# pfnet-research/superpixel-align

Measured on AMD Instinct MI355X. Metric: images/sec superpixel-align labelling (1024x2048), higher is better.
Workload: dtype f32 as 2 x f16 planes, f32 accumulate

## Files before the change

### include/spalign.h

```cpp
#ifndef SPALIGN_H
#define SPALIGN_H

#include <stddef.h>
#include <stdint.h>

#ifdef __cplusplus
extern "C" {
#endif

#define SPA_OK 0
#define SPA_ERR_ARG (-1)
#define SPA_ERR_HIP (-2)
#define SPA_ERR_NOGPU (-3)
#define SPA_ERR_LAYOUT (-4)
#define SPA_ERR_CAPACITY (-5)

#define SPA_ST_SLIC_EMPTY_SEGMENT 0x01u
#define SPA_ST_SLIC_UNCOVERED 0x02u
#define SPA_ST_CONN_OVERSIZE 0x04u
#define SPA_ST_POOL_SLOT_OVERFLOW 0x08u
#define SPA_ST_KMEANS_BARRIER 0x10u
#define SPA_ST_LABEL_RANGE 0x20u
#define SPA_ST_RNG_UNDERRUN 0x40u
#define SPA_ST_NP_SHUFFLE 0x80u

#define SPA_CELL_SLOTS 16

typedef struct spa_ctx spa_ctx;

int spa_version(void);
const char *spa_last_error(void);
int spa_ctx_create(int device, spa_ctx **out);
void spa_ctx_destroy(spa_ctx *ctx);
int spa_status(spa_ctx *ctx, uint32_t *status_host, void *stream);
int spa_status_peek_async(spa_ctx *ctx, uint32_t *status_pinned, void *stream);
int spa_status_take_async(spa_ctx *ctx, uint32_t *status_pinned, void *stream);

int spa_prof_enable(spa_ctx *ctx, int on);
int spa_prof_slots(void);
const char *spa_prof_name(int slot);
int spa_prof_read(spa_ctx *ctx, int slot, double *total_ms_host, int *launches_host);
int spa_debug_peek(spa_ctx *ctx, int which, size_t offset, size_t bytes, void *host);
int spa_ws_generation(spa_ctx *ctx);
int spa_debug_set(spa_ctx *ctx, int32_t key, int32_t value);
int spa_wino4_tile_decode(int32_t B, int32_t H, int32_t W, int32_t dilation, int32_t interleaved, int64_t t, int32_t *out);
int spa_debug_lds_probe(spa_ctx *ctx, float *out, int32_t n_wg, int32_t steps, int32_t mode, void *stream);

int spa_drn_normalise(spa_ctx *ctx, const float *x, int32_t B, int32_t H, int32_t W, void *out,
                      int32_t out_dtype, const double *mean3_host, const double *std3_host, void *stream);
int spa_bias_act(spa_ctx *ctx, void *y, int32_t dtype, int64_t rows, int32_t C, const void *bias,
                 const void *residual, int32_t relu, void *stream);
int spa_bias_act_amax(spa_ctx *ctx, float *y, int64_t rows, int32_t C, const float *bias,
                      const float *residual, int32_t relu, void *amax, void *stream);

int spa_drn_stem_d(spa_ctx *ctx, const float *x, int32_t B, int32_t H, int32_t W,
                   const float *w0, const float *b0, const float *w1, const float *b1,
                   const double *mean3_host, const double *std3_host, void *y, int32_t out_dtype,
                   float *xn_scratch, void *stream);

int spa_conv3x3_bf16(spa_ctx *ctx, const void *x, int32_t B, int32_t H, int32_t W, int32_t Cin,
                     const void *wt, int32_t Cout, const float *bias, const void *residual,
                     int32_t relu, int32_t dilation, void *y, void *stream);

int spa_conv_bf16_light(spa_ctx *ctx, const void *x, int32_t B, int32_t Hi, int32_t Wi, int32_t Cin, const void *wt,
                        int32_t taps, int32_t stride, int32_t Cout, const float *bias, const void *residual,
                        int32_t relu, int32_t dilation, void *y, void *stream);

// ... 306 lines not shown
```

### superpixel-align_amd/_lib.py

```python
import ctypes
import os
import subprocess

_HERE = os.path.dirname(os.path.abspath(__file__))
LIB_PATH = os.environ.get('SPA_LIB_PATH') or os.path.join(_HERE, 'libspalign.so')
_LIB = None

SPA_OK = 0
STATUS_BITS = {
    0x01: 'SLIC: a seed lost all of its pixels (NaN centre, dead for the rest of the sweeps, as in scikit-image)',
    0x02: 'SLIC: a pixel fell outside every 2S search window',
    0x04: 'connectivity: a component reached max_size (cut in BFS order by the exact replay path)',
    0x08: 'mean pooling: more than 16 superpixels touch one feature pixel',
    0x10: 'k-means: grid barrier timed out',
    0x20: 'a superpixel label outside [0, n_labels) was met',
    0x40: 'anchor selection: the device random stream ran dry',
    0x80: 'k-means initial assignment on the device: more than 65 536 points at or below the median weight',
}

INFO_BITS = 0x01 | 0x04

c_i32 = ctypes.c_int32
c_i64 = ctypes.c_int64
c_f32 = ctypes.c_float
# ... 35 lines not shown
    'spa_conv3x3_f32': (ctypes.c_int, [c_p, c_p, c_i32, c_i32, c_i32, c_i32, c_p, c_i32, c_p, c_p, c_i32, c_i32, c_p, c_p]),
    'spa_conv1x1_f32': (ctypes.c_int, [c_p, c_p, c_i32, c_i32, c_i32, c_i32, c_p, c_i32, c_p, c_p, c_i32, c_p, c_p]),
    'spa_wino_tiles': (ctypes.c_int64, [c_i32, c_i32, c_i32, c_i32]),
    'spa_conv3x3_wino_f32': (ctypes.c_int, [c_p, c_p, c_i32, c_i32, c_i32, c_i32, c_p, c_i32, c_p, c_p, c_i32, c_i32, c_p, c_p, c_p, c_p]),
    'spa_wino4_tiles': (ctypes.c_int64, [c_i32, c_i32, c_i32, c_i32]),
    'spa_conv3x3_wino4_f32': (ctypes.c_int, [c_p, c_p, c_i32, c_i32, c_i32, c_i32, c_p, c_i32, c_p, c_p, c_i32, c_i32, c_p, c_p, c_p, c_p]),
    'spa_conv3x3_f16s': (ctypes.c_int, [c_p, c_p, c_i32, c_i32, c_i32, c_i32, c_p, c_f32, c_i32, c_p, c_p, c_i32, c_i32, c_p, c_p, c_p, c_p]),
    'spa_conv1x1_f16s': (ctypes.c_int, [c_p, c_p, c_i32, c_i32, c_i32, c_i32, c_p, c_f32, c_i32, c_p, c_p, c_i32, c_p, c_p, c_p, c_p]),
    'spa_conv3x3_s2_f16s': (ctypes.c_int, [c_p, c_p, c_i32, c_i32, c_i32, c_i32, c_p, c_f32, c_i32, c_i32, c_p, c_i32, c_p, c_p, c_p, c_p, c_p]),
    'spa_bias_act_amax': (ctypes.c_int, [c_p, c_p, c_i64, c_i32, c_p, c_p, c_i32, c_p, c_p]),
    'spa_drn_stem_d_amax': (ctypes.c_int, [c_p, c_p, c_i32, c_i32, c_i32, c_p, c_p, c_p, c_p, c_p, c_p, c_p, c_p, c_p, c_p]),
    'spa_drn_stem_c_amax': (ctypes.c_int, [c_p, c_p, c_i32, c_i32, c_i32, c_p, c_p, c_p, c_p, c_p, c_p, c_p, c_p, c_p, c_p, c_p]),
    'spa_drn_stem_c_bf16': (ctypes.c_int, [c_p, c_p, c_i32, c_i32, c_i32, c_p, c_p, c_p, c_p, c_p, c_p, c_p, c_p, c_p, c_p]),
    'spa_conv_small_f16s': (ctypes.c_int, [c_p, c_p, c_i32, c_i32, c_i32, c_i32, c_p, c_f32, c_i32, c_i32, c_i32, c_p, c_p, c_i32, c_p, c_p, c_p, c_p, c_p]),
    'spa_drn_layer2_f16s': (ctypes.c_int, [c_p, c_p, c_i32, c_i32, c_i32, c_p, c_f32, c_p, c_p, c_p, c_p, c_p]),
    'spa_drn_layer2_f32': (ctypes.c_int, [c_p, c_p, c_i32, c_i32, c_i32, c_p, c_p, c_p, c_p]),
    'spa_conv3x3_s2_f32': (ctypes.c_int, [c_p, c_p, c_i32, c_i32, c_i32, c_i32, c_p, c_i32, c_i32, c_p, c_i32, c_p, c_p, c_p]),
    'spa_amax_f32': (ctypes.c_int, [c_p, c_p, c_i64, c_p, c_p]),
    'spa_conv3x3_wino4_f16s': (ctypes.c_int, [c_p, c_p, c_i32, c_i32, c_i32, c_i32, c_p, c_p, c_i32, c_p, c_p, c_i32, c_i32, c_p, c_p, c_p, c_p, c_p, c_p]),
    'spa_resize_bicubic_u8': (ctypes.c_int, [c_p, c_p, c_i32, c_i32, c_i32, c_i32, c_i32, c_i32, c_p, c_p]),
    'spa_resize_cvcubic_u8': (ctypes.c_int, [c_p, c_p, c_i32, c_i32, c_i32, c_i32, c_i32, c_i32, c_p, c_p]),
    'spa_debug_peek': (ctypes.c_int, [c_p, ctypes.c_int, ctypes.c_size_t, ctypes.c_size_t, c_p]),
    'spa_debug_set': (ctypes.c_int, [c_p, ctypes.c_int32, ctypes.c_int32]),
    'spa_wino4_tile_decode': (ctypes.c_int, [c_i32, c_i32, c_i32, c_i32, c_i32, c_i64, ctypes.POINTER(ctypes.c_int32)]),
    'spa_ws_generation': (ctypes.c_int, [c_p]),
    'spa_debug_lds_probe': (ctypes.c_int, [c_p, c_p, c_i32, c_i32, c_i32, c_p]),
    'spa_slic_make_plan':(ctypes.c_int, [c_i32, c_i32, c_i32, ctypes.POINTER(SlicPlan)]),
    'spa_rgb2lab': (ctypes.c_int, [c_p, c_p, c_i32, c_i32, c_i32, c_f32, c_p, c_p]),
    'spa_slic_core': (ctypes.c_int, [c_p, c_p, c_i32, c_i32, c_i32, c_i32, c_i32, c_p, c_p, c_p]),
    'spa_enforce_connectivity': (ctypes.c_int, [c_p, c_p, c_i32, c_i32, c_i32, c_i32, c_i32, c_p,
                                                c_p, c_p]),
    'spa_slic': (ctypes.c_int, [c_p, c_p, c_i32, c_i32, c_i32, c_i32, c_f32, c_i32, c_p, c_p, c_p]),
    'spa_felzenszwalb': (ctypes.c_int, [c_p, c_p, c_i32, c_i32, c_i32, c_f64, c_f64, c_i32, c_p, c_p, c_p]),
    'spa_rgb2lab_u8_f64': (ctypes.c_int, [c_p, c_p, c_i32, c_i32, c_i32, c_f64, c_p, c_p]),
    'spa_slic_core_f64': (ctypes.c_int, [c_p, c_p, c_i32, c_i32, c_i32, c_i32, c_i32, c_p, c_p, c_p]),
    'spa_slic_u8': (ctypes.c_int, [c_p, c_p, c_i32, c_i32, c_i32, c_i32, c_f64, c_i32, c_p, c_p, c_p]),
    'spa_felzenszwalb_u8': (ctypes.c_int, [c_p, c_p, c_i32, c_i32, c_i32, c_f64, c_f64, c_i32, c_p, c_p, c_p]),
    'spa_overlap_refine': (ctypes.c_int, [c_p, c_p, c_p, c_i32, c_i64, c_i32, c_f64, c_p, c_p]),
    'spa_segment_offsets':(ctypes.c_int, [c_p, c_p, c_i32, c_p, c_p]),
    'spa_segment_stats': (ctypes.c_int, [c_p, c_p, c_i32, c_i32, c_i32, c_p, c_i32, c_f64, c_f64,
                                         c_f64, c_f64, c_p, c_p, c_p, c_p]),
    'spa_pyrandom_create': (ctypes.c_int, [ctypes.c_uint64, ctypes.POINTER(c_p)]),
    'spa_pyrandom_destroy': (None, [c_p]),
    'spa_pyrandom_shuffle_select_host': (ctypes.c_int, [c_p, c_p, c_i32, c_i32, c_p, c_p]),
    'spa_nprandom_create': (ctypes.c_int, [ctypes.c_uint32, ctypes.POINTER(c_p)]),
    'spa_nprandom_destroy': (None, [c_p]),
# ... 117 lines not shown
```

### superpixel-align_amd/csrc/spa_common.h

```cpp
#pragma once
#include <hip/hip_runtime.h>
#include <stdint.h>
#include <stdio.h>
#include <string.h>

#include "../../include/spalign.h"

#define SPA_WAVE 64

void spa_set_error(const char *fmt, ...);

#define SPA_HIP(call)                                                                  \
    do {                                                                               \
        hipError_t e_ = (call);                                                        \
        if (e_ != hipSuccess) {                                                        \
            spa_set_error("%s failed: %s (%s:%d)", #call, hipGetErrorString(e_),      \
                          __FILE__, __LINE__);                                         \
            return SPA_ERR_HIP;                                                        \
        }                                                                              \
    } while (0)

#define SPA_ARG(cond)                                                                  \
    do {                                                                               \
        if (!(cond)) {                                                                 \
// ... 40 lines not shown
    WS_FZ_KEYS,
    WS_FZ_VALS,
    WS_FZ_STATE,
    WS_FZ_TMP,
    WS_STEM_WPACK,
    WS_ZERO_LINE,
    WS_RESIZE_TAB,
    WS_RESIZE_TMP,
    WS_RNG_STATE,
    WS_RNG_RING,
    WS_RNG_JBUF,
    WS_RNG_JOFF,
    WS_RUNS,
    WS_DEBUG,
    WS_SEGNET_BNPART,
    WS_SEGNET_WROT,
    WS_SEGNET_WGRAD,
    WS_SEGNET_WBF16,
    WS_SEGNET_WF16X3,
    WS_SEGNET_AMAX,
    WS_SEGNET_BNRED,
    WS_PNG_ROWS,
    WS_JPEG_INTERVALS,
    WS_COUNT
};

enum {
    PROF_RGB2LAB = 0, PROF_SLIC_ASSIGN, PROF_SLIC_UPDATE, PROF_CONNECT, PROF_STATS,
    PROF_CELL_WEIGHTS, PROF_POOL_MEAN, PROF_POOL_ANCHOR, PROF_KMEANS, PROF_PAINT,
    PROF_DRN_STEM, PROF_DRN_BIAS_ACT, PROF_DRN_CONV, PROF_DRN_CONV32, PROF_DRN_GEMM32, PROF_DRN_GEMM32_N, PROF_WINO_IN, PROF_WINO_OUT, PROF_DRN_GEMM16, PROF_DRN_GEMM16_N, PROF_DRN_CONV16, PROF_DRN_CONV16_128, PROF_DRN_CONV16_256, PROF_DRN_CONV16_1X1, PROF_DRN_CONV16_FRONT, PROF_DRN_CONV_LIGHT, PROF_SLOTS
};

struct spa_ctx {
    int device;
    int n_cu;
    uint32_t *d_status;
    unsigned status_takes;
    void *ws[WS_COUNT];
    size_t ws_bytes[WS_COUNT];
    int prof_on;
    hipEvent_t *prof_ev[PROF_SLOTS];
    int prof_cap[PROF_SLOTS], prof_used[PROF_SLOTS];
    hipStream_t aux[2];
    hipEvent_t ev_fork, ev_join[2];
    int aux_ready;
    int km_attr_done[2];
    int conn_attr_done;
    int conn_claim_ready;
    size_t conn_claim_bytes;
    int upd_wg_per_cu, upd_wg_per_cu8;
    int slic_force_general;
    int zero_line_ready, conv_attr_done, conv32_attr_done, fz_attr_done, gemm16_attr_done, gemm16s_attr_done, gemm16p_attr_done, nprng_attr_done;
    int rng_seeded;
    int ws_generation;
    int dbg_slic_ldsx;
    int convp_on;
    int wino_operands;
    int convs2_on;
    int convs2_attr_done;
    int rs_key[4], rs_ks[2];
};

#ifdef __HIPCC__
__device__ __forceinline__ unsigned spa_split16_pair(float x0, float x1, float sc, unsigned &l)
{
    unsigned h, lo;
    asm("v_fma_mixlo_f16 %0, %2, %4, 0 op_sel_hi:[0,0,0]\n\t"
        "v_fma_mixhi_f16 %0, %3, %4, 0 op_sel_hi:[0,0,0]\n\t"
        "v_fma_mixlo_f16 %1, %2, %4, -%0 op_sel_hi:[0,0,1]\n\t"
        "v_fma_mixhi_f16 %1, %3, %4, -%0 op_sel:[0,0,1] op_sel_hi:[0,0,1]"
        : "=&v"(h), "=&v"(lo) : "v"(x0), "v"(x1), "v"(sc));
    l = lo;
    return h;
}
#endif

int spa_aux_streams(spa_ctx *ctx);

void spa_prof_mark(spa_ctx *ctx, int slot, int end, hipStream_t s);
struct SpaProfScope {
    spa_ctx *c; int slot; hipStream_t s;
    SpaProfScope(spa_ctx *c_, int slot_, hipStream_t s_) : c(c_), slot(slot_), s(s_) { if (c->prof_on && slot >= 0) spa_prof_mark(c, slot, 0, s); }
// ... 65 lines not shown
```

### superpixel-align_amd/csrc/spa_ctx.hip

```cpp
#include <math.h>
#include <stdarg.h>
#include <stdlib.h>

#include "spa_common.h"

static thread_local char g_err[512] = "";

void spa_set_error(const char *fmt, ...)
{
    va_list ap;
    va_start(ap, fmt);
    vsnprintf(g_err, sizeof(g_err), fmt, ap);
    va_end(ap);
}

extern "C" const char *spa_last_error(void) { return g_err; }
extern "C" int spa_version(void) { return 100; }

extern "C" int spa_ctx_create(int device, spa_ctx **out)
{
    SPA_ARG(out != nullptr);
    int n = 0;
    if (hipGetDeviceCount(&n) != hipSuccess || n <= 0) {
        spa_set_error("no HIP device visible: libspalign has no CPU fallback");
        return SPA_ERR_NOGPU;
    }
    if (device < 0) SPA_HIP(hipGetDevice(&device));
    SPA_ARG(device < n);
    SPA_HIP(hipSetDevice(device));
    hipDeviceProp_t prop;
    SPA_HIP(hipGetDeviceProperties(&prop, device));
    if (strncmp(prop.gcnArchName, "gfx950", 6) != 0) {
        spa_set_error("device %d is %s; libspalign is built for gfx950 (MI355X) only", device,
                      prop.gcnArchName);
        return SPA_ERR_NOGPU;
    }
    spa_ctx *ctx = (spa_ctx *)calloc(1, sizeof(spa_ctx));
    ctx->device = device;
    ctx->n_cu = prop.multiProcessorCount;
    if (const char *e = getenv("SPA_SLIC_GENERAL")) ctx->slic_force_general = atoi(e) != 0;
    ctx->convp_on = getenv("SPA_CONVP") ? atoi(getenv("SPA_CONVP")) != 0 : 1;
    ctx->convs2_on = 1;
    ctx->wino_operands = 2;
    SPA_HIP(hipMalloc((void **)&ctx->d_status, 32 * sizeof(uint32_t)));
    SPA_HIP(hipMemset(ctx->d_status, 0, 32 * sizeof(uint32_t)));
    *out = ctx;
    return SPA_OK;
}

extern "C" void spa_ctx_destroy(spa_ctx *ctx)
{
    if (!ctx) return;
    for (int i = 0; i < PROF_SLOTS; ++i) {
        for (int j = 0; j < ctx->prof_cap[i]; ++j) (void)hipEventDestroy(ctx->prof_ev[i][j]);
        free(ctx->prof_ev[i]);
    }
    for (int i = 0; i < WS_COUNT; ++i)
        if (ctx->ws[i]) (void)hipFree(ctx->ws[i]);
    if (ctx->d_status) (void)hipFree(ctx->d_status);
    if (ctx->aux_ready) {
        for (int i = 0; i < 2; ++i) { (void)hipStreamDestroy(ctx->aux[i]); (void)hipEventDestroy(ctx->ev_join[i]); }
        (void)hipEventDestroy(ctx->ev_fork);
    }
    free(ctx);
}

__global__ void k_zero_word(unsigned *w) { *w = 0u; }
void spa_zero_word(void *word, hipStream_t s) { hipLaunchKernelGGL(k_zero_word, dim3(1), dim3(1), 0, s, (unsigned *)word); }

int spa_ws_reserve(spa_ctx *ctx, int which, size_t bytes, void **out)
{
    if (bytes == 0) bytes = 16;
    if (ctx->ws_bytes[which] < bytes) {
        SPA_HIP(hipDeviceSynchronize());
        if (ctx->ws[which]) SPA_HIP(hipFree(ctx->ws[which]));
        ctx->ws[which] = nullptr;
        ctx->ws_bytes[which] = 0;
        size_t want = bytes + bytes / 8;
        SPA_HIP(hipMalloc(&ctx->ws[which], want));
        ctx->ws_bytes[which] = want;
        ++ctx->ws_generation;
    }
// ... 208 lines not shown
            const bool take = best[i] > dd[i];
            best[i] = take ? dd[i] : best[i];
            bl[i] = take ? jj : bl[i];
        }
        if (p0.x < 1e30f) acc0 = p0;
        if (p1.x < 1e30f) acc1 = p1;
    }
    float4 r = make_float4(best[0] + (float)bl[0], best[1] + (float)bl[1], best[2] + (float)bl[2], best[3] + (float)bl[3]);
    *(float4 *)(out + ((long long)blockIdx.x * 256 + tid) * 4) = r;
}

extern "C" int spa_debug_lds_probe(spa_ctx *ctx, float *out, int32_t n_wg, int32_t steps, int32_t mode, void *stream)
{
    SPA_ARG(ctx && out && n_wg > 0 && steps > 0 && steps <= 32 && mode >= 0 && mode <= 2);
    hipLaunchKernelGGL(k_debug_lds_probe, dim3((unsigned)n_wg), dim3(256), 0, spa_stream(stream), out, steps, mode, 0.731f);
    SPA_LAUNCH_CHECK();
    return SPA_OK;
}

extern "C" int spa_ws_generation(spa_ctx *ctx) { return ctx ? ctx->ws_generation : -1; }

extern "C" int spa_debug_set(spa_ctx *ctx, int32_t key, int32_t value)
{
    SPA_ARG(ctx && (key == 1 || key == 2 || key == 3 || key == 4) && (value == 0 || value == 1 || (key == 4 && value == 2)));
    if (key == 1) ctx->convp_on = value;
    else if (key == 4) ctx->wino_operands = value;
    else if (key == 3) ctx->convs2_on = value;
    else {
#ifdef SPA_DIAG
        ctx->dbg_slic_ldsx = value;
#else
        SPA_ARG(!"spa_debug_set key 2 (the reproducer variant of k_slic_assign) exists in diagnostic builds only: make EXTRA=-DSPA_DIAG");
#endif
    }
    return SPA_OK;
}

extern "C" int spa_debug_peek(spa_ctx *ctx, int which, size_t offset, size_t bytes, void *host)
{
    if (which == -1) which = WS_DEBUG;
    SPA_ARG(ctx && host && which >= 0 && which < WS_COUNT && offset + bytes <= ctx->ws_bytes[which]);
    SPA_HIP(hipDeviceSynchronize());
    SPA_HIP(hipMemcpy(host, (const char *)ctx->ws[which] + offset, bytes, hipMemcpyDeviceToHost));
    return SPA_OK;
}
```

### superpixel-align_amd/csrc/spa_slic.hip

```cpp
#include "spa_common.h"
#include <stdlib.h>
#include "spa_glibcf.h"

int spa_slic_core_general_f32(spa_ctx *ctx, const float *lab, int32_t B, int32_t H, int32_t W, int32_t n_segments,
                              int32_t max_iter, int32_t *labels, float *centres, void *stream);

__device__ __forceinline__ float lab_f(float s, const spa_glibcf_tables *__restrict__ T)
{
    if (s > (float)0.008856) return spa_glibc_cbrtf(s, T);
    return (float)7.787 * s + (float)(16.0 / 116.0);
}

__device__ __forceinline__ float srgb_linear(float a, const spa_glibcf_tables *__restrict__ T)
{
    if (a > (float)0.04045) {
        float u = (a + (float)0.055) / (float)1.055;
        return spa_glibc_powf_2p4(u, T);
    }
    return a / (float)12.92;
}

__global__ void k_srgb_lut(float *__restrict__ lut)
{
    lut[threadIdx.x] = srgb_linear((float)threadIdx.x, &spa_glibcf_global);
// ... 130 lines not shown
}

__global__ void k_slic_init(uint32_t *__restrict__ cen, int nC, int grid_nx, int start_y,
                            int start_x, int step_y, int step_x, int s2y, int s2x, int H, int W)
{
    int k = blockIdx.x * blockDim.x + threadIdx.x;
    int b = blockIdx.y;
    if (k >= nC) return;
    int iy = k / grid_nx, ix = k % grid_nx;
    float cy = (float)(start_y + iy * step_y), cx = (float)(start_x + ix * step_x);
    int y0, y1, x0, x1;
    slic_window(cy, cx, s2y, s2x, H, W, y0, y1, x0, x1);
    uint32_t *c = cen + ((long long)b * nC + k) * CEN_WORDS;
    c[0] = __float_as_uint(cy); c[1] = __float_as_uint(cx);
    c[2] = 0u; c[3] = 0u; c[4] = 0u; c[5] = 0u;
    c[6] = (uint32_t)y0; c[7] = (uint32_t)y1; c[8] = (uint32_t)x0; c[9] = (uint32_t)x1;
    c[10] = 0u; c[11] = 0u;
    c[12] = 0x7fffffffu; c[13] = 0u; c[14] = 0x7fffffffu; c[15] = 0u;
}

#define TILE 32
typedef float f32x2 __attribute__((ext_vector_type(2)));

template <bool LDSX>
__global__ __launch_bounds__(256) void k_slic_assign(const float *__restrict__ lab,
                                                     uint32_t *__restrict__ cen, int nC,
                                                     int H, int W, float sw,
                                                     int32_t *__restrict__ labels,
                                                     unsigned long long *__restrict__ rowmask, int HG, int PW,
                                                     uint32_t *__restrict__ fine, int RW, int PWF,
                                                     uint32_t *__restrict__ status)
{
    __shared__ uint4 cand[256 * 3];
    __shared__ __attribute__((aligned(16))) float cdx[LDSX ? 32 * TILE : 4];
    __shared__ int wave_cnt[4];
    const int b = blockIdx.z;
    const int ty0 = blockIdx.y * TILE, tx0 = blockIdx.x * TILE;
    const int tid = threadIdx.x, lane = tid & 63, wv = tid >> 6;
    const long long npix = (long long)H * W;
    const float *pl = lab + (long long)b * 3 * npix;
    uint32_t *cb = cen + (long long)b * nC * CEN_WORDS;

    const int y = ty0 + (tid >> 3);
    const int xb = tx0 + (tid & 7) * 4;
    const bool row_ok = y < H;
    float pL[4], pA[4], pB[4];
    bool ok[4];
#pragma unroll
    for (int i = 0; i < 4; ++i) ok[i] = row_ok && (xb + i) < W;
    const long long base = (long long)y * W + xb;
    if (ok[3] && ((base & 3) == 0)) {
        float4 l4 = *(const float4 *)(pl + base);
        float4 a4 = *(const float4 *)(pl + npix + base);
        float4 b4 = *(const float4 *)(pl + 2 * npix + base);
        pL[0] = l4.x; pL[1] = l4.y; pL[2] = l4.z; pL[3] = l4.w;
        pA[0] = a4.x; pA[1] = a4.y; pA[2] = a4.z; pA[3] = a4.w;
        pB[0] = b4.x; pB[1] = b4.y; pB[2] = b4.z; pB[3] = b4.w;
    } else {
#pragma unroll
        for (int i = 0; i < 4; ++i) {
            pL[i] = ok[i] ? pl[base + i] : 0.0f;
            pA[i] = ok[i] ? pl[npix + base + i] : 0.0f;
            pB[i] = ok[i] ? pl[2 * npix + base + i] : 0.0f;
        }
    }
    float best[4] = {INFINITY, INFINITY, INFINITY, INFINITY};
    int bl[4] = {-1, -1, -1, -1};
    const float fy = (float)y;
    const f32x2 pL2[2] = {{pL[0], pL[1]}, {pL[2], pL[3]}}, pA2[2] = {{pA[0], pA[1]}, {pA[2], pA[3]}},
                pB2[2] = {{pB[0], pB[1]}, {pB[2], pB[3]}};
    const f32x2 fx2[2] = {{(float)xb, (float)(xb + 1)}, {(float)(xb + 2), (float)(xb + 3)}};

    for (int kb = 0; kb < nC; kb += 256) {
        const int k = kb + tid;
        bool hit = false;
        uint4 w0, w1, w2;
        if (k < nC) {
            const uint4 *c = (const uint4 *)(cb + (long long)k * CEN_WORDS);
            w0 = c[0]; w1 = c[1]; w2 = c[2];
            int y0 = (int)w1.z, y1 = (int)w1.w, x0 = (int)w2.x, x1 = (int)w2.y;
            hit = (y0 < ty0 + TILE) && (y1 > ty0) && (x0 < tx0 + TILE) && (x1 > tx0);
        }
        unsigned long long m = __ballot(hit);
        if (lane == 0) wave_cnt[wv] = __popcll(m);
        __syncthreads();
        int off = 0, total = 0;
#pragma unroll
        for (int i = 0; i < 4; ++i) {
            int c = wave_cnt[i];
            if (i < wv) off += c;
            total += c;
        }
        if (hit) {
            int pos = off + (int)spa_rank_in_mask(m);
            cand[pos * 3 + 0] = w0;
            cand[pos * 3 + 1] = make_uint4(w1.x, (uint32_t)k, w1.z, w1.w);
            const bool whole = (int)w1.z <= ty0 && (int)w1.w >= ty0 + TILE && (int)w2.x <= tx0 && (int)w2.y >= tx0 + TILE &&
                               ty0 + TILE <= H && tx0 + TILE <= W;
            cand[pos * 3 + 2] = make_uint4(w2.x, w2.y, whole ? 1u : 0u, 0u);
        }
        __syncthreads();
        if constexpr (LDSX) {
            for (int j0 = 0; j0 < total; j0 += 32) {
                const int jn = min(32, total - j0);
                for (int e = tid; e < jn * TILE; e += 256) {
                    const int j = j0 + (e >> 5), xi = e & 31;
                    const uint4 e0 = cand[j * 3 + 0], e2 = cand[j * 3 + 2];
                    const int xx = tx0 + xi;
                    const float t = __uint_as_float(e0.y) - (float)xx;
                    const bool in = ((unsigned)(xx - (int)e2.x) < (unsigned)((int)e2.y - (int)e2.x)) && xx < W;
                    cdx[(e >> 5) * TILE + xi] = in ? t * t : INFINITY;
                }
                __syncthreads();
                if (row_ok) {
#pragma unroll 1
                    for (int jj = 0; jj < jn; ++jj) {
                        const int j = j0 + jj;
                        const uint4 e0 = cand[j * 3 + 0], e1 = cand[j * 3 + 1];
                        const float4 dx4 = *(const float4 *)(cdx + jj * TILE + (tid & 7) * 4);
                        const int y0 = (int)e1.z, y1 = (int)e1.w;
                        const float cy = __uint_as_float(e0.x);
                        const float cl = __uint_as_float(e0.z), ca = __uint_as_float(e0.w);
// ... 5 lines not shown
                        const f32x2 dxp[2] = {{dx4.x, dx4.y}, {dx4.z, dx4.w}};
#pragma unroll
                        for (int h = 0; h < 2; ++h) {
                            f32x2 dc = (f32x2{dy, dy} + dxp[h]) * f32x2{sw, sw};
                            const f32x2 t0 = pL2[h] - f32x2{cl, cl}, t1 = pA2[h] - f32x2{ca, ca}, t2 = pB2[h] - f32x2{cbb, cbb};
                            f32x2 col = t0 * t0;
                            col = col + t1 * t1;
                            col = col + t2 * t2;
                            dc = dc + col;
#pragma unroll
                            for (int q = 0; q < 2; ++q) {
                                const int i = 2 * h + q;
                                const float d = q ? dc.y : dc.x;
                                const bool take = best[i] > d;
                                best[i] = take ? d : best[i];
                                bl[i] = take ? kk : bl[i];
                            }
                        }
                    }
                }
                __syncthreads();
            }
        } else {
            if (row_ok) {
    #pragma unroll 1
                for (int j = 0; j < total; ++j) {
                    const uint4 e0 = cand[j * 3 + 0], e1 = cand[j * 3 + 1], e2 = cand[j * 3 + 2];
                    const int y0 = (int)e1.z, y1 = (int)e1.w, x0 = (int)e2.x, x1 = (int)e2.y;
                    const float cy = __uint_as_float(e0.x), cx = __uint_as_float(e0.y);
                    const float cl = __uint_as_float(e0.z), ca = __uint_as_float(e0.w);
                    const float cbb = __uint_as_float(e1.x);
                    const int kk = (int)e1.y;
                    const float ty = cy - fy;
                    const float dy = ty * ty;
                    const bool whole = __builtin_amdgcn_readfirstlane((int)e2.z) != 0;
                    if (whole) {
    #pragma unroll
                        for (int h = 0; h < 2; ++h) {
                            const f32x2 tx = f32x2{cx, cx} - fx2[h];
                            const f32x2 dx = tx * tx;
                            f32x2 dc = (f32x2{dy, dy} + dx) * f32x2{sw, sw};
                            const f32x2 t0 = pL2[h] - f32x2{cl, cl}, t1 = pA2[h] - f32x2{ca, ca}, t2 = pB2[h] - f32x2{cbb, cbb};
                            f32x2 col = t0 * t0;
                            col = col + t1 * t1;
                            col = col + t2 * t2;
                            dc = dc + col;
    #pragma unroll
                            for (int q = 0; q < 2; ++q) {
                                const int i = 2 * h + q;
                                const float d = q ? dc.y : dc.x;
                                const bool take = best[i] > d;
                                best[i] = take ? d : best[i];
                                bl[i] = take ? kk : bl[i];
                            }
                        }
                        continue;
                    }
                    const bool rowin = (y >= y0) && (y < y1);
                    const unsigned xw = (unsigned)(x1 - x0);
    #pragma unroll
                    for (int h = 0; h < 2; ++h) {
                        const f32x2 tx = f32x2{cx, cx} - fx2[h];
                        const f32x2 dx = tx * tx;
                        f32x2 dc = (f32x2{dy, dy} + dx) * f32x2{sw, sw};
                        const f32x2 t0 = pL2[h] - f32x2{cl, cl}, t1 = pA2[h] - f32x2{ca, ca}, t2 = pB2[h] - f32x2{cbb, cbb};
                        f32x2 col = t0 * t0;
                        col = col + t1 * t1;
                        col = col + t2 * t2;
                        dc = dc + col;
    #pragma unroll
                        for (int q = 0; q < 2; ++q) {
                            const int i = 2 * h + q;
                            const float d = q ? dc.y : dc.x;
                            const bool take = rowin && ok[i] && ((unsigned)(xb + i - x0) < xw) && (best[i] > d);
                            best[i] = take ? d : best[i];
                            bl[i] = take ? kk : bl[i];
                        }
                    }
                }
            }
            __syncthreads();
        }
        }
    bool uncovered = false;
#pragma unroll
    for (int i = 0; i < 4; ++i) uncovered = uncovered || (ok[i] && bl[i] < 0);
    if (uncovered) atomicOr(status, SPA_ST_SLIC_UNCOVERED);
    if (fine) {
        bool val[4], done[4];
#pragma unroll
        for (int i = 0; i < 4; ++i) { val[i] = ok[i] && bl[i] >= 0; done[i] = !val[i]; }
        const int piece = tx0 >> 6;
        const int half = (tx0 >> 5) & 1;
        while (true) {
            const unsigned long long pend = __ballot(!(done[0] && done[1] && done[2] && done[3]));
            if (!pend) break;
            const int leader = __ffsll((long long)pend) - 1;
            const int mine = !done[0] ? bl[0] : (!done[1] ? bl[1] : (!done[2] ? bl[2] : bl[3]));
            const int ll = __shfl(mine, leader);
            unsigned long long bi[4];
#pragma unroll
            for (int i = 0; i < 4; ++i) {
                const bool m = val[i] && bl[i] == ll;
                bi[i] = __ballot(m);
                done[i] = done[i] || m;
            }
            uint32_t rowbits = 0u;
// ... 500 lines not shown
    rc = spa_ws_reserve(ctx, WS_SLIC_ORDER, ((size_t)upd_total + 8 + 32) * 4, (void **)&upd_order);
    if (rc != SPA_OK) return rc;
    int *upd_qhead = upd_order + upd_total;
    if (!ctx->upd_wg_per_cu) {
        SPA_HIP(hipFuncSetAttribute((const void *)k_slic_update2<4>, hipFuncAttributeMaxDynamicSharedMemorySize, (int)Upd2Lds<4>::bytes));
        SPA_HIP(hipFuncSetAttribute((const void *)k_slic_update2<8>, hipFuncAttributeMaxDynamicSharedMemorySize, (int)Upd2Lds<8>::bytes));
        SPA_HIP(hipOccupancyMaxActiveBlocksPerMultiprocessor(&ctx->upd_wg_per_cu, (const void *)k_slic_update2<4>,
                                                             (UPD2_NSEG + 1) * 64, Upd2Lds<4>::bytes));
        SPA_HIP(hipOccupancyMaxActiveBlocksPerMultiprocessor(&ctx->upd_wg_per_cu8, (const void *)k_slic_update2<8>,
                                                             (UPD2_NSEG + 1) * 64, Upd2Lds<8>::bytes));
        if (ctx->upd_wg_per_cu < 1) ctx->upd_wg_per_cu = 1;
        if (ctx->upd_wg_per_cu8 < 1) ctx->upd_wg_per_cu8 = 1;
    }
    const bool upd_narrow = PW <= 4 && 4 * pl.win_step_y + 24 < 2048;
    int upd_grid = (upd_narrow ? ctx->upd_wg_per_cu : ctx->upd_wg_per_cu8) * ctx->n_cu;
    if (upd_grid > (upd_total + UPD2_NSEG - 1) / UPD2_NSEG) upd_grid = (upd_total + UPD2_NSEG - 1) / UPD2_NSEG;
    upd_grid = (upd_grid + 7) & ~7;
    const unsigned mean_px = (unsigned)(((long long)H * W) / nC) ? (unsigned)(((long long)H * W) / nC) : 1u;
    hipLaunchKernelGGL(k_slic_init, dim3((nC + 127) / 128, B), dim3(128), 0, s, cen, nC,
                       pl.grid_nx, pl.start_y, pl.start_x, pl.step_y, pl.step_x, s2y, s2x, H, W);
    SPA_LAUNCH_CHECK();
    const float sw = (float)(1.0 / (double)(pl.step * pl.step));
    dim3 ga((W + TILE - 1) / TILE, (H + TILE - 1) / TILE, B);
    const int stop_after = getenv("SPA_SLIC_STOP") ? atoi(getenv("SPA_SLIC_STOP")) : 1 << 30;
    int launched = 0;
    for (int it = 0; it < max_iter; ++it) {
        if (launched >= stop_after) break;
        ++launched;
        { SpaProfScope prof_(ctx, PROF_SLIC_ASSIGN, s);
        const bool upd = it + 1 < max_iter || centres;
#ifdef SPA_DIAG
        if (ctx->dbg_slic_ldsx)
            hipLaunchKernelGGL(k_slic_assign<true>, ga, dim3(256), 0, s, lab, cen, nC, H, W, sw, labels,
                               rowmask, HG, PW, upd ? (uint32_t *)fine : (uint32_t *)nullptr, RW, PWF, ctx->d_status);
        else
#endif
        hipLaunchKernelGGL(k_slic_assign<false>, ga, dim3(256), 0, s, lab, cen, nC, H, W, sw, labels,
                           rowmask, HG, PW, upd ? (uint32_t *)fine : (uint32_t *)nullptr, RW, PWF,
                           ctx->d_status); }
        SPA_LAUNCH_CHECK();
        if (launched >= stop_after) break;
        if (it + 1 < max_iter || centres) {
            ++launched;
            SpaProfScope prof_(ctx, PROF_SLIC_UPDATE, s);
            hipLaunchKernelGGL(k_slic_order, dim3(8), dim3(1024), 0, s, cen, upd_total, upd_per_xcd, mean_px,
                               upd_order, upd_qhead);
            if (upd_narrow)
                hipLaunchKernelGGL(k_slic_update2<4>, dim3(upd_grid), dim3((UPD2_NSEG + 1) * 64), Upd2Lds<4>::bytes, s, lab, cen, nC, B,
                                   H, W, s2y, s2x, rowmask, HG, PW, fine, RW, PWF, upd_per_xcd,
                                   (const int *)upd_order, upd_qhead, ctx->d_status);
            else
                hipLaunchKernelGGL(k_slic_update2<8>, dim3(upd_grid), dim3((UPD2_NSEG + 1) * 64), Upd2Lds<8>::bytes, s, lab, cen, nC, B,
                                   H, W, s2y, s2x, rowmask, HG, PW, fine, RW, PWF, upd_per_xcd,
                                   (const int *)upd_order, upd_qhead, ctx->d_status);
            SPA_LAUNCH_CHECK();
        }
    }
    if (centres) {
        long long total = (long long)B * nC;
        hipLaunchKernelGGL(k_slic_export_centres, dim3((unsigned)((total + 255) / 256)), dim3(256),
                           0, s, cen, centres, total);
        SPA_LAUNCH_CHECK();
// ... 28 lines not shown
```

### superpixel-align_amd/engine.py

```python
import ctypes

import numpy as np
import torch

from . import _lib
from ._lib import FmapDesc, SpalignError, check


def _ptr(t):
    return ctypes.c_void_p(t.data_ptr()) if t is not None else ctypes.c_void_p(0)


def _stream(device=None):
    return ctypes.c_void_p(torch.cuda.current_stream(device).cuda_stream)


def _req(t, dtype, what):
    if not (isinstance(t, torch.Tensor) and t.is_cuda and t.dtype == dtype and t.is_contiguous()):
        raise SpalignError('%s must be a contiguous CUDA tensor of dtype %s' % (what, dtype))
    return t


def _out(out, shape, dtype, device):
    if out is None:
# ... 60 lines not shown
    def raise_on_word(self, word, ignore=_lib.INFO_BITS):
        st = int(word.item()) & 0xffffffff
        self.last_info = st & _lib.INFO_BITS
        st &= ~ignore
        if st:
            self.status()
            msgs = [m for bit, m in _lib.STATUS_BITS.items() if st & bit]
            raise SpalignError('device status 0x%x: %s' % (st, '; '.join(msgs)))

    def raise_on_status(self, ignore=_lib.INFO_BITS):
        st = self.status()
        self.last_info = st & _lib.INFO_BITS
        st &= ~ignore
        if st:
            msgs = [m for bit, m in _lib.STATUS_BITS.items() if st & bit]
            raise SpalignError('device status 0x%x: %s' % (st, '; '.join(msgs)))

    def ws_generation(self):
        return int(self._lib.spa_ws_generation(self._ctx))

    def debug_set(self, key, value):
        check(self._lib.spa_debug_set(self._ctx, int(key), int(value)))
        self.__dict__.setdefault('_debug', {})[int(key)] = int(value)

    def debug_get(self, key, default):
        return self.__dict__.get('_debug', {}).get(int(key), default)

    def prof_enable(self, on=True):
        check(self._lib.spa_prof_enable(self._ctx, 1 if on else 0))
        self._prof_on = bool(on)

    def prof_is_on(self):
        return bool(getattr(self, '_prof_on', False))

    def prof_read(self):
        out = {}
        for slot in range(self._lib.spa_prof_slots()):
            ms, n = ctypes.c_double(0), ctypes.c_int(0)
            check(self._lib.spa_prof_read(self._ctx, slot, ctypes.byref(ms), ctypes.byref(n)))
            if n.value:
                out[self._lib.spa_prof_name(slot).decode()] = (ms.value, n.value)
        return out

    def drn_normalise(self, x, dtype=torch.float32):
        x = _req(x, torch.float32, 'x')
        B, C, H, W = x.shape
# ... 1182 lines not shown
```

Before: 450.7.

## Prune SLIC assignment candidates using per-wave colour bounding boxes

Adds a pruned variant of the SLIC assign kernel. Each wave computes a Lab colour bounding box of its pixels on the first iteration and caches it in a workspace table. Per candidate centre, a lower bound on the distance is derived from the box and a spatial clamp. After seeding with the best candidate, only candidates whose bound is at or below the wave's current worst-best distance are evaluated. This cuts distance evaluations in the assign loop at the cost of extra LDS, bound computation and a box table; the path is on by default, with an optional counter mode for diagnostics.

```diff
diff --git a/include/spalign.h b/include/spalign.h
--- a/include/spalign.h
+++ b/include/spalign.h
@@ -43,6 +43,7 @@
 int spa_debug_peek(spa_ctx *ctx, int which, size_t offset, size_t bytes, void *host);
 int spa_ws_generation(spa_ctx *ctx);
 int spa_debug_set(spa_ctx *ctx, int32_t key, int32_t value);
+int spa_slic_prune_counters(spa_ctx *ctx, uint64_t *listed_evaluated_host, int32_t reset);
 int spa_wino4_tile_decode(int32_t B, int32_t H, int32_t W, int32_t dilation, int32_t interleaved, int64_t t, int32_t *out);
 int spa_debug_lds_probe(spa_ctx *ctx, float *out, int32_t n_wg, int32_t steps, int32_t mode, void *stream);
 
diff --git a/superpixel-align_amd/_lib.py b/superpixel-align_amd/_lib.py
--- a/superpixel-align_amd/_lib.py
+++ b/superpixel-align_amd/_lib.py
@@ -81,6 +81,7 @@
     'spa_resize_cvcubic_u8': (ctypes.c_int, [c_p, c_p, c_i32, c_i32, c_i32, c_i32, c_i32, c_i32, c_p, c_p]),
     'spa_debug_peek': (ctypes.c_int, [c_p, ctypes.c_int, ctypes.c_size_t, ctypes.c_size_t, c_p]),
     'spa_debug_set': (ctypes.c_int, [c_p, ctypes.c_int32, ctypes.c_int32]),
+    'spa_slic_prune_counters': (ctypes.c_int, [c_p, ctypes.POINTER(ctypes.c_uint64), ctypes.c_int32]),
     'spa_wino4_tile_decode': (ctypes.c_int, [c_i32, c_i32, c_i32, c_i32, c_i32, c_i64, ctypes.POINTER(ctypes.c_int32)]),
     'spa_ws_generation': (ctypes.c_int, [c_p]),
     'spa_debug_lds_probe': (ctypes.c_int, [c_p, c_p, c_i32, c_i32, c_i32, c_p]),
diff --git a/superpixel-align_amd/csrc/spa_common.h b/superpixel-align_amd/csrc/spa_common.h
--- a/superpixel-align_amd/csrc/spa_common.h
+++ b/superpixel-align_amd/csrc/spa_common.h
@@ -86,6 +86,7 @@
     WS_SEGNET_BNRED,
     WS_PNG_ROWS,
     WS_JPEG_INTERVALS,
+    WS_SLIC_BOX,
     WS_COUNT
 };
 
@@ -122,6 +123,8 @@
     int wino_operands;
     int convs2_on;
     int convs2_attr_done;
+    int slic_prune;
+    unsigned long long *d_slic_cnt;
     int rs_key[4], rs_ks[2];
 };
 
diff --git a/superpixel-align_amd/csrc/spa_ctx.hip b/superpixel-align_amd/csrc/spa_ctx.hip
--- a/superpixel-align_amd/csrc/spa_ctx.hip
+++ b/superpixel-align_amd/csrc/spa_ctx.hip
@@ -42,6 +42,9 @@
     ctx->convp_on = getenv("SPA_CONVP") ? atoi(getenv("SPA_CONVP")) != 0 : 1;
     ctx->convs2_on = 1;
     ctx->wino_operands = 2;
+    ctx->slic_prune = 1;
+    SPA_HIP(hipMalloc((void **)&ctx->d_slic_cnt, 2 * sizeof(unsigned long long)));
+    SPA_HIP(hipMemset(ctx->d_slic_cnt, 0, 2 * sizeof(unsigned long long)));
     SPA_HIP(hipMalloc((void **)&ctx->d_status, 32 * sizeof(uint32_t)));
     SPA_HIP(hipMemset(ctx->d_status, 0, 32 * sizeof(uint32_t)));
     *out = ctx;
@@ -58,6 +61,7 @@
     for (int i = 0; i < WS_COUNT; ++i)
         if (ctx->ws[i]) (void)hipFree(ctx->ws[i]);
     if (ctx->d_status) (void)hipFree(ctx->d_status);
+    if (ctx->d_slic_cnt) (void)hipFree(ctx->d_slic_cnt);
     if (ctx->aux_ready) {
         for (int i = 0; i < 2; ++i) { (void)hipStreamDestroy(ctx->aux[i]); (void)hipEventDestroy(ctx->ev_join[i]); }
         (void)hipEventDestroy(ctx->ev_fork);
@@ -312,8 +316,9 @@
 
 extern "C" int spa_debug_set(spa_ctx *ctx, int32_t key, int32_t value)
 {
-    SPA_ARG(ctx && (key == 1 || key == 2 || key == 3 || key == 4) && (value == 0 || value == 1 || (key == 4 && value == 2)));
+    SPA_ARG(ctx && key >= 1 && key <= 5 && (value == 0 || value == 1 || ((key == 4 || key == 5) && value == 2)));
     if (key == 1) ctx->convp_on = value;
+    else if (key == 5) ctx->slic_prune = value;
     else if (key == 4) ctx->wino_operands = value;
     else if (key == 3) ctx->convs2_on = value;
     else {
@@ -326,6 +331,15 @@
     return SPA_OK;
 }
 
+extern "C" int spa_slic_prune_counters(spa_ctx *ctx, uint64_t *listed_evaluated_host, int32_t reset)
+{
+    SPA_ARG(ctx && listed_evaluated_host);
+    SPA_HIP(hipDeviceSynchronize());
+    SPA_HIP(hipMemcpy(listed_evaluated_host, ctx->d_slic_cnt, 2 * sizeof(uint64_t), hipMemcpyDeviceToHost));
+    if (reset) SPA_HIP(hipMemset(ctx->d_slic_cnt, 0, 2 * sizeof(uint64_t)));
+    return SPA_OK;
+}
+
 extern "C" int spa_debug_peek(spa_ctx *ctx, int which, size_t offset, size_t bytes, void *host)
 {
     if (which == -1) which = WS_DEBUG;
diff --git a/superpixel-align_amd/csrc/spa_slic.hip b/superpixel-align_amd/csrc/spa_slic.hip
--- a/superpixel-align_amd/csrc/spa_slic.hip
+++ b/superpixel-align_amd/csrc/spa_slic.hip
@@ -176,18 +176,101 @@
 #define TILE 32
 typedef float f32x2 __attribute__((ext_vector_type(2)));
 
-template <bool LDSX>
+enum { RED_MIN = 0, RED_MAX = 1 };
+template <int OP>
+__device__ __forceinline__ uint32_t slic_wave_reduce(uint32_t v)
+{
+#define SLIC_RED_STEP(ctrl)                                                                        \
+    { const uint32_t o = (uint32_t)__builtin_amdgcn_update_dpp(0, (int)v, ctrl, 0xF, 0xF, true);   \
+      v = OP == RED_MAX ? max(v, o) : min(v, o); }
+    SLIC_RED_STEP(0xB1) SLIC_RED_STEP(0x4E) SLIC_RED_STEP(0x141) SLIC_RED_STEP(0x140)
+#undef SLIC_RED_STEP
+    const uint32_t r0 = (uint32_t)__builtin_amdgcn_readlane((int)v, 0), r1 = (uint32_t)__builtin_amdgcn_readlane((int)v, 16);
+    const uint32_t r2 = (uint32_t)__builtin_amdgcn_readlane((int)v, 32), r3 = (uint32_t)__builtin_amdgcn_readlane((int)v, 48);
+    return OP == RED_MAX ? max(max(r0, r1), max(r2, r3)) : min(min(r0, r1), min(r2, r3));
+}
+__device__ __forceinline__ uint32_t slic_ord(float f)
+{
+    const uint32_t b = __float_as_uint(f);
+    return b ^ ((uint32_t)((int32_t)b >> 31) | 0x80000000u);
+}
+__device__ __forceinline__ float slic_unord(uint32_t k)
+{
+    return __uint_as_float(k ^ ((k & 0x80000000u) ? 0x80000000u : 0xffffffffu));
+}
+#define SLIC_EVAL_ENTRY(j) \
+                    const uint4 e0 = cand[j * 3 + 0], e1 = cand[j * 3 + 1], e2 = cand[j * 3 + 2];                                 \
+                    const int y0 = (int)e1.z, y1 = (int)e1.w, x0 = (int)e2.x, x1 = (int)e2.y;                                     \
+                    const float cy = __uint_as_float(e0.x), cx = __uint_as_float(e0.y);                                           \
+                    const float cl = __uint_as_float(e0.z), ca = __uint_as_float(e0.w);                                           \
+                    const float cbb = __uint_as_float(e1.x);                                                                      \
+                    const int kk = (int)e1.y;                                                                                     \
+                    const float ty = cy - fy;                                                                                     \
+                    const float dy = ty * ty;                                                                                     \
+                    const bool whole = __builtin_amdgcn_readfirstlane((int)e2.z) != 0;                                            \
+                    if (whole) {                                                                                                  \
+    _Pragma("unroll")                                                                                                             \
+                        for (int h = 0; h < 2; ++h) {                                                                             \
+                            const f32x2 tx = f32x2{cx, cx} - fx2[h];                                                              \
+                            const f32x2 dx = tx * tx;                                                                             \
+                            f32x2 dc = (f32x2{dy, dy} + dx) * f32x2{sw, sw};                                                      \
+                            const f32x2 t0 = pL2[h] - f32x2{cl, cl}, t1 = pA2[h] - f32x2{ca, ca}, t2 = pB2[h] - f32x2{cbb, cbb};  \
+                            f32x2 col = t0 * t0;                                                                                  \
+                            col = col + t1 * t1;                                                                                  \
+                            col = col + t2 * t2;                                                                                  \
+                            dc = dc + col;                                                                                        \
+    _Pragma("unroll")                                                                                                             \
+                            for (int q = 0; q < 2; ++q) {                                                                         \
+                                const int i = 2 * h + q;                                                                          \
+                                const float d = q ? dc.y : dc.x;                                                                  \
+                                const bool take = best[i] > d;                                                                    \
+                                best[i] = take ? d : best[i];                                                                     \
+                                bl[i] = take ? kk : bl[i];                                                                        \
+                            }                                                                                                     \
+                        }                                                                                                         \
+                        continue;                                                                                                 \
+                    }                                                                                                             \
+                    const bool rowin = (y >= y0) && (y < y1);                                                                     \
+                    const unsigned xw = (unsigned)(x1 - x0);                                                                      \
+    _Pragma("unroll")                                                                                                             \
+                    for (int h = 0; h < 2; ++h) {                                                                                 \
+                        const f32x2 tx = f32x2{cx, cx} - fx2[h];                                                                  \
+                        const f32x2 dx = tx * tx;                                                                                 \
+                        f32x2 dc = (f32x2{dy, dy} + dx) * f32x2{sw, sw};                                                          \
+                        const f32x2 t0 = pL2[h] - f32x2{cl, cl}, t1 = pA2[h] - f32x2{ca, ca}, t2 = pB2[h] - f32x2{cbb, cbb};      \
+                        f32x2 col = t0 * t0;                                                                                      \
+                        col = col + t1 * t1;                                                                                      \
+                        col = col + t2 * t2;                                                                                      \
+                        dc = dc + col;                                                                                            \
+    _Pragma("unroll")                                                                                                             \
+                        for (int q = 0; q < 2; ++q) {                                                                             \
+                            const int i = 2 * h + q;                                                                              \
+                            const float d = q ? dc.y : dc.x;                                                                      \
+                            const bool take = rowin && ok[i] && ((unsigned)(xb + i - x0) < xw) && (best[i] > d);                  \
+                            best[i] = take ? d : best[i];                                                                         \
+                            bl[i] = take ? kk : bl[i];                                                                            \
+                        }                                                                                                         \
+                    }
+#define SLIC_BOX_WORDS 8
+
+template <bool LDSX, bool PRUNE>
 __global__ __launch_bounds__(256) void k_slic_assign(const float *__restrict__ lab,
                                                      uint32_t *__restrict__ cen, int nC,
                                                      int H, int W, float sw,
                                                      int32_t *__restrict__ labels,
                                                      unsigned long long *__restrict__ rowmask, int HG, int PW,
                                                      uint32_t *__restrict__ fine, int RW, int PWF,
-                                                     uint32_t *__restrict__ status)
-{
+                                                     uint32_t *__restrict__ status,
+                                                     float *__restrict__ boxtab, int box_first,
+                                                     unsigned long long *__restrict__ cnt)
+{
+    static_assert(!(LDSX && PRUNE), "the reproducer variant keeps the full walk");
     __shared__ uint4 cand[256 * 3];
     __shared__ __attribute__((aligned(16))) float cdx[LDSX ? 32 * TILE : 4];
     __shared__ int wave_cnt[4];
+    __shared__ float box[6][4];
+    __shared__ __attribute__((aligned(16))) uint32_t lbt[4][256];
+    __shared__ __attribute__((aligned(16))) uint32_t seedk[4][4];
     const int b = blockIdx.z;
     const int ty0 = blockIdx.y * TILE, tx0 = blockIdx.x * TILE;
     const int tid = threadIdx.x, lane = tid & 63, wv = tid >> 6;
@@ -225,6 +308,49 @@
                 pB2[2] = {{pB[0], pB[1]}, {pB[2], pB[3]}};
     const f32x2 fx2[2] = {{(float)xb, (float)(xb + 1)}, {(float)(xb + 2), (float)(xb + 3)}};
 
+    const int wvu = __builtin_amdgcn_readfirstlane(wv);
+    bool box_ok = false;
+    int n_listed = 0, n_eval = 0;
+    if constexpr (PRUNE) {
+        float *rec = boxtab + ((((long long)b * gridDim.y + blockIdx.y) * gridDim.x + blockIdx.x) * 4 + wvu) * SLIC_BOX_WORDS;
+        float lo[3], hi[3];
+        if (box_first) {
+#pragma unroll
+            for (int c = 0; c < 3; ++c) { lo[c] = INFINITY; hi[c] = -INFINITY; }
+#pragma unroll
+            for (int i = 0; i < 4; ++i) {
+                if (ok[i]) {
+                    lo[0] = fminf(lo[0], pL[i]); hi[0] = fmaxf(hi[0], pL[i]);
+                    lo[1] = fminf(lo[1], pA[i]); hi[1] = fmaxf(hi[1], pA[i]);
+                    lo[2] = fminf(lo[2], pB[i]); hi[2] = fmaxf(hi[2], pB[i]);
+                }
+            }
+            box_ok = true;
+#pragma unroll
+            for (int c = 0; c < 3; ++c) {
+                lo[c] = slic_unord(slic_wave_reduce<RED_MIN>(slic_ord(lo[c])));
+                hi[c] = slic_unord(slic_wave_reduce<RED_MAX>(slic_ord(hi[c])));
+                box_ok = box_ok && fabsf(lo[c]) < INFINITY && fabsf(hi[c]) < INFINITY;
+            }
+            if (lane == 0) {
+                ((float4 *)rec)[0] = make_float4(lo[0], hi[0], lo[1], hi[1]);
+                ((float4 *)rec)[1] = make_float4(lo[2], hi[2], box_ok ? 1.0f : 0.0f, 0.0f);
+            }
+        } else {
+            const uint32_t v = __float_as_uint(rec[lane & (SLIC_BOX_WORDS - 1)]);
+#pragma unroll
+            for (int c = 0; c < 3; ++c) {
+                lo[c] = __uint_as_float(__builtin_amdgcn_readlane(v, 2 * c));
+                hi[c] = __uint_as_float(__builtin_amdgcn_readlane(v, 2 * c + 1));
+            }
+            box_ok = __builtin_amdgcn_readlane(v, 6) != 0u;
+        }
+        if (lane == 0) {
+#pragma unroll
+            for (int c = 0; c < 3; ++c) { box[2 * c][wvu] = lo[c]; box[2 * c + 1][wvu] = hi[c]; }
+        }
+    }
+
     for (int kb = 0; kb < nC; kb += 256) {
         const int k = kb + tid;
         bool hit = false;
@@ -252,6 +378,40 @@
             const bool whole = (int)w1.z <= ty0 && (int)w1.w >= ty0 + TILE && (int)w2.x <= tx0 && (int)w2.y >= tx0 + TILE &&
                                ty0 + TILE <= H && tx0 + TILE <= W;
             cand[pos * 3 + 2] = make_uint4(w2.x, w2.y, whole ? 1u : 0u, 0u);
+        }
+        if constexpr (PRUNE) {
+            if (m != 0ull) {
+                const int pos = off + (int)spa_rank_in_mask(m);
+                const bool whole = hit && (int)w1.z <= ty0 && (int)w1.w >= ty0 + TILE && (int)w2.x <= tx0 && (int)w2.y >= tx0 + TILE &&
+                                   ty0 + TILE <= H && tx0 + TILE <= W;
+                float cy = 0.0f, cx = 0.0f, cl = 0.0f, ca = 0.0f, cbb = 0.0f;
+                if (hit) {
+                    cy = __uint_as_float(w0.x); cx = __uint_as_float(w0.y);
+                    cl = __uint_as_float(w0.z); ca = __uint_as_float(w0.w); cbb = __uint_as_float(w1.x);
+                }
+                const float tx = cx - fminf(fmaxf(rintf(cx), (float)tx0), (float)(min(tx0 + TILE, W) - 1));
+                const float dx = tx * tx;
+                const float ry = rintf(cy);
+#pragma unroll 1
+                for (int w = 0; w < 4; ++w) {
+                    const float ty = cy - fminf(fmaxf(ry, (float)(ty0 + 8 * w)), (float)(min(ty0 + 8 * w + 8, H) - 1));
+                    const float dy = ty * ty;
+                    float dc = (dy + dx) * sw;
+                    const float t0 = fminf(fmaxf(cl, box[0][w]), box[1][w]) - cl;
+                    const float t1 = fminf(fmaxf(ca, box[2][w]), box[3][w]) - ca;
+                    const float t2 = fminf(fmaxf(cbb, box[4][w]), box[5][w]) - cbb;
+                    float col = t0 * t0;
+                    col = col + t1 * t1;
+                    col = col + t2 * t2;
+                    dc = dc + col;
+                    const uint32_t lbb = dc == dc ? __float_as_uint(dc) : 0u;
+                    if (hit) lbt[w][pos] = lbb;
+                    const uint32_t key = slic_wave_reduce<RED_MIN>(whole && dc < INFINITY ? ((lbb & ~0xffu) | (uint32_t)pos) : ~0u);
+                    if (lane == 0) seedk[w][wvu] = key;
+                }
+            } else if (lane < 4) {
+                seedk[lane][wvu] = ~0u;
+            }
         }
         __syncthreads();
         if constexpr (LDSX) {
@@ -303,67 +463,66 @@
                 __syncthreads();
             }
         } else {
-            if (row_ok) {
-    #pragma unroll 1
-                for (int j = 0; j < total; ++j) {
-                    const uint4 e0 = cand[j * 3 + 0], e1 = cand[j * 3 + 1], e2 = cand[j * 3 + 2];
-                    const int y0 = (int)e1.z, y1 = (int)e1.w, x0 = (int)e2.x, x1 = (int)e2.y;
-                    const float cy = __uint_as_float(e0.x), cx = __uint_as_float(e0.y);
-                    const float cl = __uint_as_float(e0.z), ca = __uint_as_float(e0.w);
-                    const float cbb = __uint_as_float(e1.x);
-                    const int kk = (int)e1.y;
-                    const float ty = cy - fy;
-                    const float dy = ty * ty;
-                    const bool whole = __builtin_amdgcn_readfirstlane((int)e2.z) != 0;
-                    if (whole) {
-    #pragma unroll
-                        for (int h = 0; h < 2; ++h) {
-                            const f32x2 tx = f32x2{cx, cx} - fx2[h];
-                            const f32x2 dx = tx * tx;
-                            f32x2 dc = (f32x2{dy, dy} + dx) * f32x2{sw, sw};
-                            const f32x2 t0 = pL2[h] - f32x2{cl, cl}, t1 = pA2[h] - f32x2{ca, ca}, t2 = pB2[h] - f32x2{cbb, cbb};
-                            f32x2 col = t0 * t0;
-                            col = col + t1 * t1;
-                            col = col + t2 * t2;
-                            dc = dc + col;
-    #pragma unroll
-                            for (int q = 0; q < 2; ++q) {
-                                const int i = 2 * h + q;
-                                const float d = q ? dc.y : dc.x;
-                                const bool take = best[i] > d;
-                                best[i] = take ? d : best[i];
-                                bl[i] = take ? kk : bl[i];
-                            }
-                        }
-                        continue;
+            if constexpr (PRUNE) {
+                n_listed += total;
+                uint32_t ub = 0x7f800000u;
+                {
+                    const uint4 sk = *(const uint4 *)seedk[wvu];
+                    const uint32_t k0 = __builtin_amdgcn_readfirstlane(sk.x), k1 = __builtin_amdgcn_readfirstlane(sk.y);
+                    const uint32_t k2 = __builtin_amdgcn_readfirstlane(sk.z), k3 = __builtin_amdgcn_readfirstlane(sk.w);
+                    const uint32_t key = min(min(k0, k1), min(k2, k3));
+                    const float sb[4] = {best[0], best[1], best[2], best[3]};
+                    const int sl[4] = {bl[0], bl[1], bl[2], bl[3]};
+                    if (key != ~0u) {
+                        const int j = (int)(key & 0xffu);
+                        do { SLIC_EVAL_ENTRY(j) } while (0);
+                        ++n_eval;
                     }
-                    const bool rowin = (y >= y0) && (y < y1);
-                    const unsigned xw = (unsigned)(x1 - x0);
-    #pragma unroll
-                    for (int h = 0; h < 2; ++h) {
-                        const f32x2 tx = f32x2{cx, cx} - fx2[h];
-                        const f32x2 dx = tx * tx;
-                        f32x2 dc = (f32x2{dy, dy} + dx) * f32x2{sw, sw};
-                        const f32x2 t0 = pL2[h] - f32x2{cl, cl}, t1 = pA2[h] - f32x2{ca, ca}, t2 = pB2[h] - f32x2{cbb, cbb};
-                        f32x2 col = t0 * t0;
-                        col = col + t1 * t1;
-                        col = col + t2 * t2;
-                        dc = dc + col;
-    #pragma unroll
-                        for (int q = 0; q < 2; ++q) {
-                            const int i = 2 * h + q;
-                            const float d = q ? dc.y : dc.x;
-                            const bool take = rowin && ok[i] && ((unsigned)(xb + i - x0) < xw) && (best[i] > d);
-                            best[i] = take ? d : best[i];
-                            bl[i] = take ? kk : bl[i];
+                    uint32_t mx = 0u;
+#pragma unroll
+                    for (int i = 0; i < 4; ++i) {
+                        mx = max(mx, ok[i] ? __float_as_uint(best[i]) : 0u);
+                        best[i] = sb[i]; bl[i] = sl[i];
+                    }
+                    if (box_ok) ub = slic_wave_reduce<RED_MAX>(mx);
+                }
+                for (int j0 = 0; j0 < total; j0 += 64) {
+                    const int jn = min(64, total - j0);
+                    unsigned long long live = 0ull;
+                    for (int q = 0; q < jn; q += 8) {
+                        const uint4 a = *(const uint4 *)&lbt[wvu][j0 + q], c = *(const uint4 *)&lbt[wvu][j0 + q + 4];
+                        const uint32_t v[8] = {a.x, a.y, a.z, a.w, c.x, c.y, c.z, c.w};
+                        uint32_t bits = 0u;
+#pragma unroll
+                        for (int t = 0; t < 8; ++t) bits |= ((uint32_t)__builtin_amdgcn_readfirstlane(v[t]) <= ub ? 1u : 0u) << t;
+                        live |= (unsigned long long)bits << q;
+                    }
+                    if (jn < 64) live &= (1ull << jn) - 1ull;
+                    n_eval += __popcll(live);
+                    if (row_ok) {
+                        while (live) {
+                            const int j = j0 + __ffsll((long long)live) - 1;
+                            live &= live - 1ull;
+                            SLIC_EVAL_ENTRY(j)
                         }
                     }
                 }
+            } else {
+                if (row_ok) {
+    #pragma unroll 1
+                    for (int j = 0; j < total; ++j) { SLIC_EVAL_ENTRY(j) }
+                }
             }
             __syncthreads();
         }
         }
     bool uncovered = false;
+    if constexpr (PRUNE) {
+        if (cnt && lane == 0 && row_ok) {
+            atomicAdd(cnt, (unsigned long long)n_listed);
+            atomicAdd(cnt + 1, (unsigned long long)n_eval);
+        }
+    }
 #pragma unroll
     for (int i = 0; i < 4; ++i) uncovered = uncovered || (ok[i] && bl[i] < 0);
     if (uncovered) atomicOr(status, SPA_ST_SLIC_UNCOVERED);
@@ -910,6 +1069,9 @@
     SPA_LAUNCH_CHECK();
     const float sw = (float)(1.0 / (double)(pl.step * pl.step));
     dim3 ga((W + TILE - 1) / TILE, (H + TILE - 1) / TILE, B);
+    float *boxtab;
+    rc = spa_ws_reserve(ctx, WS_SLIC_BOX, (size_t)ga.x * ga.y * ga.z * 4 * SLIC_BOX_WORDS * sizeof(float), (void **)&boxtab);
+    if (rc != SPA_OK) return rc;
     const int stop_after = getenv("SPA_SLIC_STOP") ? atoi(getenv("SPA_SLIC_STOP")) : 1 << 30;
     int launched = 0;
     for (int it = 0; it < max_iter; ++it) {
@@ -919,13 +1081,20 @@
         const bool upd = it + 1 < max_iter || centres;
 #ifdef SPA_DIAG
         if (ctx->dbg_slic_ldsx)
-            hipLaunchKernelGGL(k_slic_assign<true>, ga, dim3(256), 0, s, lab, cen, nC, H, W, sw, labels,
-                               rowmask, HG, PW, upd ? (uint32_t *)fine : (uint32_t *)nullptr, RW, PWF, ctx->d_status);
+            hipLaunchKernelGGL((k_slic_assign<true, false>), ga, dim3(256), 0, s, lab, cen, nC, H, W, sw, labels,
+                               rowmask, HG, PW, upd ? (uint32_t *)fine : (uint32_t *)nullptr, RW, PWF, ctx->d_status,
+                               (float *)nullptr, 0, (unsigned long long *)nullptr);
         else
 #endif
-        hipLaunchKernelGGL(k_slic_assign<false>, ga, dim3(256), 0, s, lab, cen, nC, H, W, sw, labels,
-                           rowmask, HG, PW, upd ? (uint32_t *)fine : (uint32_t *)nullptr, RW, PWF,
-                           ctx->d_status); }
+        if (ctx->slic_prune)
+            hipLaunchKernelGGL((k_slic_assign<false, true>), ga, dim3(256), 0, s, lab, cen, nC, H, W, sw, labels,
+                               rowmask, HG, PW, upd ? (uint32_t *)fine : (uint32_t *)nullptr, RW, PWF,
+                               ctx->d_status, boxtab, it == 0 ? 1 : 0,
+                               ctx->slic_prune == 2 ? ctx->d_slic_cnt : (unsigned long long *)nullptr);
+        else
+            hipLaunchKernelGGL((k_slic_assign<false, false>), ga, dim3(256), 0, s, lab, cen, nC, H, W, sw, labels,
+                               rowmask, HG, PW, upd ? (uint32_t *)fine : (uint32_t *)nullptr, RW, PWF,
+                               ctx->d_status, (float *)nullptr, 0, (unsigned long long *)nullptr); }
         SPA_LAUNCH_CHECK();
         if (launched >= stop_after) break;
         if (it + 1 < max_iter || centres) {
diff --git a/superpixel-align_amd/engine.py b/superpixel-align_amd/engine.py
--- a/superpixel-align_amd/engine.py
+++ b/superpixel-align_amd/engine.py
@@ -106,6 +106,11 @@
     def debug_set(self, key, value):
         check(self._lib.spa_debug_set(self._ctx, int(key), int(value)))
         self.__dict__.setdefault('_debug', {})[int(key)] = int(value)
+
+    def slic_prune_counters(self, reset=True):
+        out = (ctypes.c_uint64 * 2)()
+        check(self._lib.spa_slic_prune_counters(self._ctx, out, 1 if reset else 0))
+        return int(out[0]), int(out[1])
 
     def debug_get(self, key, default):
         return self.__dict__.get('_debug', {}).get(int(key), default)
```

New measurement: 445.2. 0.988x the previous value.
